# kopacja/rho2sdf.jl

Measured on NVIDIA B200. Metric: sdf_voxels_per_sec, higher is better.
Workload: dtype f64

## Files before the change

### include/r2s.h

```cpp
#ifndef R2S_H
#define R2S_H
#include <stddef.h>
#include <stdint.h>
#ifdef __cplusplus
extern "C" {
#endif

typedef struct r2s_ctx r2s_ctx;

typedef struct r2s_params {
  double rho_t;
  double delta_factor;
  int32_t remove_artifacts;
  double artifact_threshold;
  double artifact_min_ratio;
  int32_t rbf_interp;
  int32_t smooth;
  double rbf_cut;
  double target_volume;
  int32_t final_volume;
} r2s_params;

typedef struct r2s_report {
  int64_t n_solid, n_crossing, n_active, n_pairs, n_not_converged, n_newton_iters;
  int64_t n_flipped;
  int32_t cg_iters, bisections;
  float th, volume;
  float ms_bin, ms_project, ms_assemble, ms_sign, ms_cc, ms_rbf_prep, ms_cg, ms_lsf, ms_threshold, ms_fine, ms_volume, ms_total;
  int64_t launches;
  int64_t collectives;
  float cg_probe[4];
  int64_t n_pairs_pruned;
  float ms_solve, ms_scan;
} r2s_report;

int r2s_create(r2s_ctx **ctx, int device, void *stream);
void r2s_destroy(r2s_ctx *ctx);
const char *r2s_last_error(r2s_ctx *ctx);
void r2s_default_params(r2s_params *p);
int r2s_last_report(r2s_ctx *ctx, r2s_report *rep);

int r2s_set_mesh(r2s_ctx *ctx, int nen, int64_t nnp, const double *X, int64_t nel, const int64_t *IEN);
int r2s_set_grid(r2s_ctx *ctx, const double amin[3], const double amax[3], const int64_t N[3], double cell_size);

int r2s_mesh_volume(r2s_ctx *ctx, const double *rho_e, double *V_domain, double *V_frac);
int r2s_nodal_densities(r2s_ctx *ctx, const double *rho_e, double *rho_n);
int r2s_isocontour_volume(r2s_ctx *ctx, const double *rho_n, double threshold, double *volume);
int r2s_find_threshold(r2s_ctx *ctx, const double *rho_n, double target_volume, double rtol, int maxit, double *rho_t);

int r2s_eval_distances(r2s_ctx *ctx, const double *rho_n, double rho_t, double delta_factor, double *dist, double *xp);
int r2s_sign_detection(r2s_ctx *ctx, const double *rho_n, double rho_t, double *signs);
int r2s_remove_artifacts(r2s_ctx *ctx, double *sdf, double threshold, double min_component_ratio, int64_t *flipped);
int r2s_rbf_smoothing(r2s_ctx *ctx, const double *sdf, int is_interp, int smooth, double rbf_cut, double target_volume,
                      float *fine_sdf, float *th, float *volume);
int r2s_volume_from_sdf(r2s_ctx *ctx, const float *sdf, int64_t nx, int64_t ny, int64_t nz, float edge, float iso, int quad_order, double *volume);

int r2s_pipeline(r2s_ctx *ctx, const r2s_params *p, const double *rho_n, double *sdf_dists, float *fine_sdf, r2s_report *rep);
int r2s_upload_nodal_densities(r2s_ctx *ctx, const double *rho_n);
int r2s_pipeline_resident(r2s_ctx *ctx, const r2s_params *p, r2s_report *rep);
int r2s_download_sdf(r2s_ctx *ctx, double *sdf_dists);
int r2s_download_fine_sdf(r2s_ctx *ctx, float *fine_sdf);
int r2s_result_ptrs_dev(r2s_ctx *ctx, void **sdf_dev, void **fine_sdf_dev);

// ... 41 lines not shown
```

### rho2sdf.jl_b200/__init__.py

```python
import ctypes as C
import math
import os

import numpy as np

__all__ = ["HEX8", "TET4", "Rho2sdfOptions", "Mesh", "Grid", "getMesh_AABB", "generateGridPoints", "noninteractive_sdf_grid_setup",
           "DenseInNodes", "find_threshold_for_volume", "calculate_isocontour_volume", "evalDistances", "Sign_Detection",
           "remove_sdf_artifacts", "RBFs_smoothing", "calculate_volume_from_sdf", "rho2sdf", "rho2sdf_hex8", "rho2sdf_tet4",
           "exportSdfToVTI", "export_device_result_to_vti", "read_vti", "read_pvti", "MultiContext", "FineGrid", "R2SError", "slab_partition", "init_slab_comm", "broadcast_unique_id", "load_library", "library_path", "Params", "Report", "Context"]

_HERE = os.path.dirname(os.path.abspath(__file__))
_LIB = None


class R2SError(RuntimeError):
    pass


class HEX8:
    nen = 8


class TET4:
    nen = 4


class Params(C.Structure):
    _fields_ = [("rho_t", C.c_double), ("delta_factor", C.c_double), ("remove_artifacts", C.c_int32), ("artifact_threshold", C.c_double),
                ("artifact_min_ratio", C.c_double), ("rbf_interp", C.c_int32), ("smooth", C.c_int32), ("rbf_cut", C.c_double),
# ... 70 lines not shown
    L.r2s_multi_context.restype = vp
    L.r2s_multi_set_mesh.argtypes = [vp, C.c_int, C.c_int64, vp, C.c_int64, vp]
    L.r2s_multi_set_grid.argtypes = [vp, vp, vp, vp, C.c_double]
    L.r2s_multi_slab_planes.argtypes = [vp, vp]
    L.r2s_multi_set_rebalance.argtypes = [vp, C.c_int]
    L.r2s_multi_pipeline.argtypes = [vp, C.POINTER(Params), vp, vp, vp, C.POINTER(Report)]
    L.r2s_multi_export_vti.argtypes = [vp, C.c_char_p, C.c_char_p, C.c_int]
    L.r2s_pin_host.argtypes = [vp, C.c_size_t]
    L.r2s_unpin_host.argtypes = [vp]
    L.r2s_write_vti_host.argtypes = [C.c_char_p, C.c_char_p, vp, C.c_int, C.c_int64, C.c_int64, C.c_int64, vp, vp]
    L.r2s_measure_fma_peak.argtypes = [vp, C.c_int, dp]
    _LIB = L
    return L


def _f64(a):
    return np.ascontiguousarray(a, dtype=np.float64)


def _ptr(a):
    return a.ctypes.data_as(C.c_void_p)


class _BorrowedContext:

    def __init__(self, lib, h):
        self.lib, self.h = lib, C.c_void_p(h)

    def check(self, rc):
        if rc != 0:
            raise R2SError(self.lib.r2s_last_error(self.h).decode())

    def close(self):
        pass

    def report(self):
        r = Report()
        self.lib.r2s_last_report(self.h, C.byref(r))
        return r


class MultiContext:

    def __init__(self, devices):
        self.lib = load_library()
        self.h = C.c_void_p()
        ids = (C.c_int * len(devices))(*[int(d) for d in devices])
        rc = self.lib.r2s_multi_create(C.byref(self.h), ids, len(devices))
        if rc != 0 or not self.h:
            raise R2SError("r2s_multi_create failed (rc=%d): no usable CUDA device / no peer access -- this library has no CPU fallback" % rc)
        self.n = len(devices)

    def check(self, rc):
        if rc != 0:
            raise R2SError(self.lib.r2s_multi_last_error(self.h).decode())

    def slab(self, r=0):
        return _BorrowedContext(self.lib, self.lib.r2s_multi_context(self.h, int(r)))

    def slab_planes(self):
        cuts = np.zeros(self.n + 1, dtype=np.int64)
        self.check(self.lib.r2s_multi_slab_planes(self.h, _ptr(cuts)))
# ... 20 lines not shown
        if rc != 0 or not self.h:
            raise R2SError("r2s_create failed (rc=%d): no usable CUDA device -- this library has no CPU fallback" % rc)
        self._keep = []

    def check(self, rc):
        if rc != 0:
            raise R2SError(self.lib.r2s_last_error(self.h).decode())

    def close(self):
        if self.h:
            self.lib.r2s_destroy(self.h)
            self.h = C.c_void_p()

    def __del__(self):
        try:
            self.close()
        except Exception:
            pass

    def report(self):
        r = Report()
        self.lib.r2s_last_report(self.h, C.byref(r))
        return r


def slab_partition(nz_points, world, plane_cost=None, min_planes=3):
    nz_points, world = int(nz_points), int(world)
    if world < 1 or nz_points < world * (min_planes if world > 1 else 1):
        raise R2SError("cannot cut %d planes into %d slabs" % (nz_points, world))
    if plane_cost is None:
        base, rem = divmod(nz_points, world)
        out, k = [], 0
        for r in range(world):
            n = base + (1 if r < rem else 0)
            out.append((k, k + n))
            k += n
        return out
    c = np.maximum(np.asarray(plane_cost, dtype=np.float64), 1e-12)
    if c.shape != (nz_points,):
        raise R2SError("plane_cost must have one entry per plane")
    cum = np.concatenate([[0.0], np.cumsum(c)])
    cuts = [0]
    for r in range(1, world):
        k = int(np.searchsorted(cum, cum[-1] * r / world))
        k = max(k, cuts[-1] + min_planes)
        k = min(k, nz_points - (world - r) * min_planes)
# ... 380 lines not shown
```

### rho2sdf.jl_b200/csrc/r2s_api.cu

```cuda
#include <math.h>
#include <stdlib.h>
#include <string.h>
#include <new>
#include "r2s_common.cuh"


extern "C" {

int r2s_create(r2s_ctx **out, int device, void *stream) {
  if (!out) return 1;
  *out = nullptr;
  int ndev = 0;
  if (cudaGetDeviceCount(&ndev) != cudaSuccess || ndev == 0 || device < 0 || device >= ndev) return 2;
  r2s_ctx *ctx = new (std::nothrow) r2s_ctx();
  if (!ctx) return 3;
  ctx->device = device;
  memset(&ctx->rep, 0, sizeof(ctx->rep));
  if (cudaSetDevice(device) != cudaSuccess) { delete ctx; return 4; }
  if (stream) { ctx->stream = (cudaStream_t)stream; ctx->own_stream = false; }
  else { if (cudaStreamCreateWithFlags(&ctx->stream, cudaStreamNonBlocking) != cudaSuccess) { delete ctx; return 5; } ctx->own_stream = true; }
  for (int i = 0; i < 16; i++) cudaEventCreate(&ctx->ev[i]);
  for (int i = 0; i < 5; i++) { cudaEventCreate(&ctx->ev_probe[i]); cudaEventCreate(&ctx->ev_k[i]); }
  cudaStreamCreateWithFlags(&ctx->copy_stream, cudaStreamNonBlocking);
  for (int i = 0; i < 64; i++) cudaEventCreateWithFlags(&ctx->ev_copy[i], cudaEventDisableTiming);
// ... 12 lines not shown
  r2s_comm_destroy(ctx);
  DevBuf *all[] = {&ctx->X, &ctx->IEN32, &ctx->ine_ptr, &ctx->ine_el, &ctx->fbnd, &ctx->ezr, &ctx->ebox, &ctx->rho_e, &ctx->rho_n, &ctx->gtab_d, &ctx->gtab_i, &ctx->cls, &ctx->act_flag,
                   &ctx->act_idx, &ctx->act_rec, &ctx->cnt_a, &ctx->cnt_b, &ctx->keys, &ctx->keys_alt, &ctx->tile_ptr, &ctx->tile_faces, &ctx->face_tiles, &ctx->fc_list, &ctx->tri_cnt, &ctx->tri_rec, &ctx->pairbuf, &ctx->pairxp, &ctx->cubtmp,
                   &ctx->counters, &ctx->box_rec, &ctx->plist, &ctx->dist, &ctx->xp, &ctx->sdf, &ctx->signs, &ctx->s_rng, &ctx->s_el, &ctx->s_cnt, &ctx->s_keys, &ctx->s_keys_alt, &ctx->s_tile_ptr,
                   &ctx->cc_label, &ctx->cc_size, &ctx->cc_scal, &ctx->cc_bits, &ctx->cc_bits_all, &ctx->cc_gsz, &ctx->cc_seen, &ctx->f_s, &ctx->f_w, &ctx->f_r, &ctx->f_u, &ctx->f_c, &ctx->f_lsf, &ctx->f_fine, &ctx->f_part,
                   &ctx->f_scal, &ctx->cutlist, &ctx->slablist, &ctx->v_part, &ctx->vlist[0], &ctx->vlist[1], &ctx->vent[0], &ctx->vent[1], &ctx->vrec, &ctx->bis_state, &ctx->lat_xs, &ctx->lat_cell, &ctx->lat_map, &ctx->lat_info, &ctx->lat_pt};
  for (DevBuf *b : all) b->release();
  for (int i = 0; i < 16; i++) cudaEventDestroy(ctx->ev[i]);
  for (int i = 0; i < 5; i++) { cudaEventDestroy(ctx->ev_probe[i]); cudaEventDestroy(ctx->ev_k[i]); }
  for (int i = 0; i < 64; i++) cudaEventDestroy(ctx->ev_copy[i]);
  for (int i = 0; i < 2; i++) cudaEventDestroy(ctx->ev_done[i]);
  if (ctx->copy_stream) cudaStreamDestroy(ctx->copy_stream);
  if (ctx->rb_host) cudaFreeHost(ctx->rb_host);
  if (ctx->own_stream) cudaStreamDestroy(ctx->stream);
  delete ctx;
}
const char *r2s_last_error(r2s_ctx *ctx) { return ctx ? ctx->err.c_str() : "r2s: no context (no CUDA device?)"; }

void r2s_default_params(r2s_params *p) {
  p->rho_t = 0.5; p->delta_factor = 1.1; p->remove_artifacts = 1; p->artifact_threshold = 0.0; p->artifact_min_ratio = 0.01;
  p->rbf_interp = 1; p->smooth = 1; p->rbf_cut = 1e-3; p->target_volume = 0.0; p->final_volume = 1;
}
int r2s_last_report(r2s_ctx *ctx, r2s_report *rep) { if (!ctx || !rep) return 1; *rep = ctx->rep; return 0; }

int r2s_set_mesh(r2s_ctx *ctx, int nen, int64_t nnp, const double *X, int64_t nel, const int64_t *IEN) {
  if (!ctx) return 1;
  if (nen != 8 && nen != 4) FAIL("r2s_set_mesh: nen must be 8 (HEX8) or 4 (TET4)");
  if (nnp <= 0 || nel <= 0 || !X || !IEN) FAIL("r2s_set_mesh: empty mesh");
  if (nel * nen >= (1ll << 31) || nnp >= (1ll << 31)) FAIL("r2s_set_mesh: mesh too large for 32-bit connectivity");
  CK(cudaSetDevice(ctx->device));
  for (i64 t = 0; t < nel * nen; t++) if (IEN[t] < 1 || IEN[t] > nnp) FAIL("r2s_set_mesh: IEN entry out of range (expected 1-based node ids)");
  ctx->have_sdf = ctx->have_fine = false;
  ctx->nen = nen; ctx->nes = nen == 8 ? 6 : 4; ctx->nsn = nen == 8 ? 4 : 3; ctx->nnp = nnp; ctx->nel = nel;
  CK(ctx->X.reserve(sizeof(double) * 3 * (size_t)nnp));
  CK(ctx->IEN32.reserve(sizeof(int) * (size_t)(nel * nen)));
  CK(cudaMemcpyAsync(ctx->X.p, X, sizeof(double) * 3 * (size_t)nnp, cudaMemcpyHostToDevice, ctx->stream));
  if (r2s_mesh_upload_ien(ctx, IEN)) return 1;
  CK(ctx->rho_e.reserve(sizeof(double) * (size_t)nel));
  CK(ctx->rho_n.reserve(sizeof(double) * (size_t)nnp));
  if (r2s_mesh_build_tables(ctx)) return 1;
  return r2s_mesh_build_lattice(ctx);
}

int r2s_set_grid(r2s_ctx *ctx, const double amin[3], const double amax[3], const int64_t N[3], double cell) {
  if (!ctx) return 1;
  CK(cudaSetDevice(ctx->device));
// ... 300 lines not shown
```

### rho2sdf.jl_b200/csrc/r2s_common.cuh

```cuda
#pragma once
#include <cuda_runtime.h>
#include <stdint.h>
#include <stdio.h>
#include <string>
#include <vector>
#include "../../include/r2s.h"

typedef long long i64;
typedef unsigned long long u64;

#define R2S_BIG 1.0e10

#define TILE_X 8
#define TILE_Y 8
#define TILE_Z 4
#define TILE_VOX (TILE_X * TILE_Y * TILE_Z)

struct DevBuf {
  void *p = nullptr;
  size_t cap = 0;
  cudaError_t reserve(size_t bytes) {
    if (bytes <= cap) return cudaSuccess;
    if (p) cudaFree(p);
    p = nullptr; cap = 0;
// ... 58 lines not shown
  i64 nnp = 0, nel = 0;
  DevBuf X, IEN32, ine_ptr, ine_el, fbnd, ezr;
  DevBuf ebox; i64 n_box = 0;
  bool lattice = false; int lat_nd[3] = {0, 0, 0}, lat_off[3] = {0, 0, 0}; i64 lat_ncell = 0;
  DevBuf lat_xs, lat_cell, lat_map, lat_info, lat_pt;
  DevBuf rho_e, rho_n;

  bool has_grid = false;
  GridDev g;
  i64 k0 = 0, k1 = 0;
  const float *skip_flag = nullptr;
  LocalGroup *lg = nullptr;
  void *comm = nullptr; int rank = 0, nranks = 1; i64 collectives = 0; std::vector<int> slab_k0;
  bool p2p = false; void *p2p_box = nullptr; void *p2p_peer_box[64]; void **p2p_peer_box_dev = nullptr; unsigned p2p_seq = 0;
  void *p2p_c_local = nullptr; void *p2p_c_peer[2] = {nullptr, nullptr}; unsigned p2p_halo_seq = 0; i64 p2p_ops = 0;
  DevBuf gtab_d, gtab_i;
  std::vector<double> h_pc[3];

  DevBuf cls, act_flag, act_idx, act_rec, cnt_a, cnt_b, keys, keys_alt, tile_ptr, tile_faces, face_tiles, fc_list, tri_cnt, tri_rec, pairbuf, pairxp, cubtmp, counters, box_rec, plist;
  DevBuf dist, xp, sdf, signs;
  DevBuf s_rng, s_el, s_cnt, s_keys, s_keys_alt, s_tile_ptr;
  DevBuf cc_label, cc_size, cc_scal, cc_bits, cc_bits_all, cc_gsz, cc_seen;
  DevBuf f_s, f_w, f_r, f_u, f_c, f_lsf, f_fine, f_part, f_scal, cutlist, slablist, vlist[2], vent[2], vrec, bis_state;
  int smooth_last = 1;
  bool have_sdf = false, have_fine = false;

  DevBuf v_part;
};

#define CK(call)                                                                                   \
  do {                                                                                             \
    cudaError_t _e = (call);                                                                       \
    if (_e != cudaSuccess) {                                                                       \
      char _b[512];                                                                                \
      snprintf(_b, sizeof(_b), "%s:%d: %s -> %s", __FILE__, __LINE__, #call, cudaGetErrorString(_e)); \
      ctx->err = _b;                                                                               \
      return 1;                                                                                    \
    }                                                                                              \
  } while (0)

#define FAIL(msg)           \
  do {                      \
    ctx->err = (msg);       \
    return 1;               \
  } while (0)

// ... 70 lines not shown
```

### rho2sdf.jl_b200/csrc/r2s_rbf.cu

```cuda
#include <float.h>
#include <stdlib.h>
#include <algorithm>
#include <cuda.h>
#include "r2s_common.cuh"
#include "r2s_tables.cuh"
#include "r2s_p2p.cuh"
#include "r2s_volq.cuh"

__global__ void __launch_bounds__(256) k_to_f32(i64 n, i64 v0, int nx, int px, const double *__restrict__ sdf, float *__restrict__ s, unsigned *__restrict__ maxbits) {
  __shared__ float red[8];
  float a = -1.0f;
  const i64 row0 = v0 / nx;
  for (i64 v = blockIdx.x * (i64)blockDim.x + threadIdx.x; v < n; v += (i64)gridDim.x * blockDim.x) {
    const i64 row = v / nx; const int i = (int)(v - row * nx);
    float f = (float)sdf[v0 + v]; s[(row0 + row) * px + i] = f; float af = fabsf(f); if (af < 1.0e9f) a = fmaxf(a, af);
  }
  for (int o = 16; o > 0; o >>= 1) a = fmaxf(a, __shfl_down_sync(0xffffffffu, a, o));
  if ((threadIdx.x & 31) == 0) red[threadIdx.x >> 5] = a;
  __syncthreads();
  if (threadIdx.x == 0) {
    for (int i = 1; i < 8; i++) a = fmaxf(a, red[i]);
    if (a >= 0.0f) atomicMax(maxbits, __float_as_uint(a) + 1u);
  }
}
// ... 279 lines not shown
  for (i64 v = blockIdx.x * (i64)blockDim.x + threadIdx.x; v < n; v += (i64)gridDim.x * blockDim.x) s += (double)a[v] * (double)a[v];
  for (int o = 16; o > 0; o >>= 1) s += __shfl_down_sync(0xffffffffu, s, o);
  if ((threadIdx.x & 31) == 0) red[threadIdx.x >> 5] = s;
  __syncthreads();
  if (threadIdx.x == 0) { double t = 0; for (int i = 0; i < (int)(blockDim.x >> 5); i++) t += red[i]; partial[blockIdx.x] = t; }
}

__global__ void __launch_bounds__(256) k_minmax(i64 n, int nx, int px, const float *__restrict__ a, unsigned *__restrict__ mm) {
  __shared__ float rlo[8], rhi[8];
  float lo = INFINITY, hi = -INFINITY;
  for (i64 v = blockIdx.x * (i64)blockDim.x + threadIdx.x; v < n; v += (i64)gridDim.x * blockDim.x) { if ((int)(v % px) < nx) { float x = a[v]; lo = fminf(lo, x); hi = fmaxf(hi, x); } }
  for (int o = 16; o > 0; o >>= 1) { lo = fminf(lo, __shfl_down_sync(0xffffffffu, lo, o)); hi = fmaxf(hi, __shfl_down_sync(0xffffffffu, hi, o)); }
  if ((threadIdx.x & 31) == 0) { rlo[threadIdx.x >> 5] = lo; rhi[threadIdx.x >> 5] = hi; }
  __syncthreads();
  if (threadIdx.x == 0) {
    for (int i = 1; i < 8; i++) { lo = fminf(lo, rlo[i]); hi = fmaxf(hi, rhi[i]); }
    unsigned bl = __float_as_uint(lo), bh = __float_as_uint(hi);
    bl = (bl & 0x80000000u) ? ~bl : (bl | 0x80000000u); bh = (bh & 0x80000000u) ? ~bh : (bh | 0x80000000u);
    atomicMin(&mm[0], bl); atomicMax(&mm[1], bh);
  }
}
static inline float ordered_to_float(unsigned b) { b = (b & 0x80000000u) ? (b & 0x7fffffffu) : ~b; float f; memcpy(&f, &b, 4); return f; }

__device__ __forceinline__ void vol_sum_flush(u64 local, u64 *__restrict__ acc) {
  __shared__ u64 s_w[2][8];
  u64 s[2] = {local & 0xffffffffull, local >> 32};
  for (int o = 16; o > 0; o >>= 1) { s[0] += __shfl_down_sync(0xffffffffu, s[0], o); s[1] += __shfl_down_sync(0xffffffffu, s[1], o); }
  if ((threadIdx.x & 31) == 0) { s_w[0][threadIdx.x >> 5] = s[0]; s_w[1][threadIdx.x >> 5] = s[1]; }
  __syncthreads();
  if (threadIdx.x == 0) {
    u64 a = 0, b = 0;
    for (int w = 0; w < (int)(blockDim.x >> 5); w++) { a += s_w[0][w]; b += s_w[1][w]; }
    if (a) atomicAdd(&acc[2], a);
    if (b) atomicAdd(&acc[7], b);
  }
}
__global__ void __launch_bounds__(128) k_vol_cut(int nx, int ny, int px, const float *__restrict__ sdf, float th, float iso, const int *__restrict__ cutlist, int cutcap,
                                                 GaussF G, u64 *__restrict__ acc) {
  const int ncut = (int)min((u64)cutcap, acc[1]);
  const int nthr = gridDim.x * blockDim.x;
  const i64 sxy = (i64)px * ny;
  u64 local = 0;
  for (int base = blockIdx.x * blockDim.x; base < ncut; base += nthr) {
    const int idx = base + threadIdx.x;
    if (idx < ncut) {
      const i64 c = cutlist[idx];
// ... 139 lines not shown
    int cutcap = (int)(ctx->cutlist.cap / sizeof(int));
    CK(cudaMemsetAsync(acc, 0, sizeof(u64) * 8, st));
    vol_march<false>(st, nx, ny, px, 0, nz - 1, sdf, iso, iso, iso, nullptr, nullptr, 0, acc, ctx->cutlist.as<int>(), cutcap); LAUNCH_CHECK();
    if (order == 9) k_vol_cut<<<148 * 16, 128, 0, st>>>(nx, ny, px, sdf, 0.0f, iso, ctx->cutlist.as<int>(), cutcap, G9, acc);
    else {
      GaussTab t = gauss_legendre_host(order); GaussNF G; G.n = order;
      for (int q = 0; q < 32; q++) { G.x[q] = q < order ? (float)t.x[q] : 0.0f; G.w[q] = q < order ? (float)t.w[q] : 0.0f; }
      k_vol_cut_n<<<148 * 16, 128, 0, st>>>(nx, ny, px, sdf, 0.0f, iso, ctx->cutlist.as<int>(), cutcap, G, acc);
    }
    LAUNCH_CHECK();
    u64 h[8];
    if (r2s_readback(ctx, h, acc, sizeof(h))) return 1;
    if ((i64)h[1] > cutcap) {
      CK(ctx->cutlist.reserve(sizeof(int) * (size_t)(h[1] + h[1] / 2 + 1024)));
      continue;
    }
    float ev = edge * edge * edge, jac = ev / 8.0f;
    *vol = (double)h[0] * (double)ev + vol_fixed_value(h[2], h[7]) * (double)jac;
    return 0;
  }
  FAIL("calculate_volume_from_sdf: cut-cell list overflow");
}
struct VRec { float c[8]; };
struct VCache { float part, th_e, margin; int pad; };
struct BisState {
  float lo, hi, th, th_prev; int nb, have_prev, done, skip; float skipf; int cur; double v, eps, target; float ev, jac; unsigned long long n_eval;
};
__device__ __forceinline__ void bis_begin(BisState *S, u64 *acc) {
  if (S->done) { S->skip = 1; S->skipf = 1.0f; return; }
  const float th = (S->lo + S->hi) / 2;
  S->th = th;
  const int skip = (S->have_prev && th == S->th_prev) ? 1 : 0;
  S->skip = skip; S->skipf = skip ? 1.0f : 0.0f;
  if (!skip) { acc[0] = 0; acc[1] = 0; acc[2] = 0; acc[7] = 0; acc[4 + (1 - S->cur)] = 0; }
}
__device__ __forceinline__ void bis_end(BisState *S, const u64 *acc, const u64 *red) {
  if (S->done) return;
  if (!S->skip) {
    S->v = fma((double)red[0], (double)S->ev, __dmul_rn(vol_fixed_value(red[2], red[3]), (double)S->jac));
    S->cur = 1 - S->cur; S->n_eval += acc[1];
  }
  const float cur = (float)S->v;
  S->eps = fabs(S->target - (double)cur);
  if ((double)cur > S->target) S->lo = S->th; else S->hi = S->th;
  S->nb++; S->have_prev = 1; S->th_prev = S->th;
  if (!(S->nb < 40 && S->eps > 1.0e-4)) S->done = 1;
}
#define VL_U 4
__global__ void __launch_bounds__(256) k_vl_step(const BisState *__restrict__ S, VAct *l0, VAct *l1, i64 out_cap, int use_cache, u64 *__restrict__ acc, const VCache *__restrict__ cache,
                                                 int2 *__restrict__ evlist, i64 ev_cap) {
  if (S->skip) return;
  const int icur = S->cur;
  const VAct *__restrict__ in = icur ? l1 : l0; VAct *__restrict__ out = icur ? l0 : l1;
  const u64 *n_in_ptr = acc + 4 + icur; u64 *n_out_ptr = acc + 4 + (1 - icur);
  const float lo = S->lo, hi = S->hi, th = S->th;
  __shared__ VAct s_keep[8][WS_CAP];
  __shared__ int2 s_ev[8][WS_CAP];
  const i64 n_in = (i64)*n_in_ptr;
  const int lane = threadIdx.x & 31, warp = threadIdx.x >> 5;
  int nfull = 0, nperm = 0, nkq = 0, neq = 0; u64 local = 0;
  for (i64 t0 = ((i64)blockIdx.x * blockDim.x + (threadIdx.x & ~31)) * VL_U; t0 < n_in; t0 += (i64)gridDim.x * blockDim.x * VL_U) {
    VAct e[VL_U];
#pragma unroll
    for (int u = 0; u < VL_U; u++) {
      const i64 t = t0 + u * 32 + lane;
      if (t < n_in) { const int4 q = __ldcs(reinterpret_cast<const int4 *>(in) + t); e[u].id = q.x; e[u].mn = __int_as_float(q.y); e[u].mx = __int_as_float(q.z); e[u].rec = q.w; }
      else { e[u].id = 0; e[u].mn = INFINITY; e[u].mx = INFINITY; e[u].rec = -1; }
    }
    float4 r[VL_U];
#pragma unroll
    for (int u = 0; u < VL_U; u++) {
      r[u] = make_float4(0.f, 0.f, 0.f, 0.f);
      const bool cached = use_cache && e[u].rec >= 0 && !(e[u].mn >= hi) && !(e[u].mx < lo) && !(e[u].mx < th) && !(e[u].mn >= th);
      if (cached) r[u] = __ldg(reinterpret_cast<const float4 *>(cache) + e[u].rec);
    }
#pragma unroll
    for (int u = 0; u < VL_U; u++) {
      const bool valid = t0 + u * 32 + lane < n_in;
      bool keep = false, miss = false, fresh = false;
      if (valid) {
        if (e[u].mn >= hi) nperm++;
        else if (e[u].mx < lo) {}
        else {
          keep = true;
          if (!(e[u].mx < th)) {
            if (e[u].mn >= th) nfull++;
            else if (e[u].rec < 0) { miss = true; fresh = true; }
            else if (use_cache && fabsf(th - r[u].y) * 1.00001f < r[u].z) vol_cell_add(local, r[u].x);
            else miss = true;
          }
        }
      }
      const unsigned mf = __ballot_sync(0xffffffffu, fresh);
      if (mf) {
        int base = 0;
        if (lane == 0) base = (int)atomicAdd(&acc[6], (u64)__popc(mf));
        base = __shfl_sync(0xffffffffu, base, 0);
        if (fresh) e[u].rec = base + __popc(mf & ((1u << lane) - 1));
      }
      ws_push<VAct>(s_keep[warp], nkq, keep, e[u], out, n_out_ptr, out_cap, lane);
      ws_push<int2>(s_ev[warp], neq, miss, make_int2(e[u].rec | (fresh ? (int)0x80000000 : 0), e[u].id), evlist, &acc[1], ev_cap, lane);
    }
  }
  ws_flush<VAct>(s_keep[warp], nkq, out, n_out_ptr, out_cap, lane);
  ws_flush<int2>(s_ev[warp], neq, evlist, &acc[1], ev_cap, lane);
  for (int o = 16; o > 0; o >>= 1) { nfull += __shfl_down_sync(0xffffffffu, nfull, o); nperm += __shfl_down_sync(0xffffffffu, nperm, o); }
  if (lane == 0) { if (nfull) atomicAdd(&acc[0], (u64)nfull); if (nperm) atomicAdd(&acc[3], (u64)nperm); }
  vol_sum_flush(local, acc);
}
__global__ void __launch_bounds__(128) k_vl_eval(const BisState *__restrict__ S, VRec *__restrict__ recs, VCache *__restrict__ cache, const int2 *__restrict__ evlist, int nx, int ny,
                                                 int px, const float *__restrict__ sdf, GaussF G, u64 *__restrict__ acc) {
  if (S->skip) return;
  const float th = S->th;
  const int nev = (int)acc[1];
  const int nthr = gridDim.x * blockDim.x;
  u64 local = 0;
  for (int base = blockIdx.x * blockDim.x; base < nev; base += nthr) {
    const int idx = base + threadIdx.x;
    if (idx < nev) {
      const int2 q = evlist[idx];
      VRec &e = recs[q.x & 0x7fffffff];
      float c[8];
      if (q.x < 0) {
        const i64 cpl = (i64)(nx - 1) * (ny - 1), sxy = (i64)px * ny;
        const int i = q.y % (nx - 1), j = (q.y / (nx - 1)) % (ny - 1), k = (int)(q.y / cpl);
        const i64 b = ((i64)k * ny + j) * px + i;
        c[0] = sdf[b]; c[1] = sdf[b + 1]; c[2] = sdf[b + px]; c[3] = sdf[b + px + 1];
        c[4] = sdf[b + sxy]; c[5] = sdf[b + sxy + 1]; c[6] = sdf[b + sxy + px]; c[7] = sdf[b + sxy + px + 1];
        float4 *d = reinterpret_cast<float4 *>(e.c);
        d[0] = make_float4(c[0], c[1], c[2], c[3]); d[1] = make_float4(c[4], c[5], c[6], c[7]);
      } else {
        const float4 *d = reinterpret_cast<const float4 *>(e.c), a = d[0], b = d[1];
        c[0] = a.x; c[1] = a.y; c[2] = a.z; c[3] = a.w; c[4] = b.x; c[5] = b.y; c[6] = b.z; c[7] = b.w;
      }
#pragma unroll
      for (int a = 0; a < 8; a++) c[a] = c[a] - th;
      const float amax = fmaxf(fmaxf(fmaxf(fabsf(c[0]), fabsf(c[1])), fmaxf(fabsf(c[2]), fabsf(c[3]))), fmaxf(fmaxf(fabsf(c[4]), fabsf(c[5])), fmaxf(fabsf(c[6]), fabsf(c[7]))));
      float m;
      const float part = cut_cell_quad9<true>(c, G, 0.0f, &m);
      VCache w; w.part = part; w.th_e = th; w.margin = m - 1.0e-5f * amax; w.pad = 0;
      cache[q.x & 0x7fffffff] = w;
      vol_cell_add(local, part);
    }
  }
  vol_sum_flush(local, acc);
}
__device__ __forceinline__ void vol_pack(const u64 *__restrict__ acc, int cutcap, u64 *__restrict__ red, const BisState *S) {
  if (S && S->skip) return;
  red[0] = acc[0] + acc[3]; red[1] = acc[1] > (u64)cutcap ? 1 : 0; red[2] = acc[2]; red[3] = acc[7];
}
__global__ void k_vol_pack(const u64 *__restrict__ acc, int cutcap, u64 *__restrict__ red, const BisState *S) { vol_pack(acc, cutcap, red, S); }
__global__ void k_bis_turn(BisState *S, u64 *acc, u64 *red, int what) {
  if (what & 4) vol_pack(acc, 0x7fffffff, red, S);
  if (what & 2) bis_end(S, acc, red);
  if (what & 1) bis_begin(S, acc);
}
struct VolBisect {
  const float *sdf; int nx, ny, px, kc0, kc1; float edge; int step, cur; i64 n_cur, n_eval; u64 *acc;
};
static int vol_bisect_begin(r2s_ctx *ctx, VolBisect &vb, const float *sdf, int nx, int ny, int nz, int px, int kc0, int kc1, float edge) {
  i64 ncell = (i64)(nx - 1) * (ny - 1) * (nz - 1);
  if (ncell >= (1ll << 31)) FAIL("LS_Threshold: grid too large for 32-bit cell ids");
  CK(ctx->f_scal.reserve(512));
  vb.sdf = sdf; vb.nx = nx; vb.ny = ny; vb.px = px; vb.kc0 = kc0; vb.kc1 = kc1; vb.edge = edge; vb.step = 0; vb.cur = 0; vb.n_eval = 0;
  vb.n_cur = (i64)(nx - 1) * (ny - 1) * (i64)(kc1 - kc0);
  vb.acc = (u64 *)((char *)ctx->f_scal.p + 128);
  CK(cudaMemsetAsync(vb.acc, 0, sizeof(u64) * 12, ctx->stream));
  return 0;
}
static int vol_bisect_step(r2s_ctx *ctx, VolBisect &vb, float lo, float hi, float th, double *vol) {
  cudaStream_t st = ctx->stream;
  static const GaussF G9 = gauss9f();
  const i64 n_all = (i64)(vb.nx - 1) * (vb.ny - 1) * (i64)(vb.kc1 - vb.kc0);
  vb.step++;
  const bool emit = vb.step == 3;
  if (emit) CK(ctx->vent[0].reserve(sizeof(VAct) * (size_t)(n_all + 1)));
  u64 h[6];
  for (int attempt = 0; attempt < 2; attempt++) {
    int cutcap = (int)(ctx->cutlist.cap / sizeof(int));
    CK(cudaMemsetAsync(vb.acc, 0, sizeof(u64) * 8, st));
    u64 *nout = vb.acc + 4;
    if (!emit) vol_march<false>(st, vb.nx, vb.ny, vb.px, vb.kc0, vb.kc1, vb.sdf, lo, hi, th, nullptr, nullptr, 0, vb.acc, ctx->cutlist.as<int>(), cutcap);
    else vol_march<true>(st, vb.nx, vb.ny, vb.px, vb.kc0, vb.kc1, vb.sdf, lo, hi, th, ctx->vent[0].as<VAct>(), nout, n_all + 1, vb.acc, ctx->cutlist.as<int>(), cutcap);
    LAUNCH_CHECK();
    k_vol_cut<<<148 * 16, 128, 0, st>>>(vb.nx, vb.ny, vb.px, vb.sdf, th, 0.0f, ctx->cutlist.as<int>(), cutcap, G9, vb.acc); LAUNCH_CHECK();
    u64 *red = vb.acc + 8, hr[4];
    k_vol_pack<<<1, 1, 0, st>>>(vb.acc, cutcap, red, nullptr); LAUNCH_CHECK();
    if (r2s_allreduce(ctx, red, 4, 1)) return 1;
    {
      u64 hall[12];
      if (r2s_readback(ctx, hall, vb.acc, sizeof(hall))) return 1;
      for (int q = 0; q < 6; q++) h[q] = hall[q];
      for (int q = 0; q < 4; q++) hr[q] = hall[8 + q];
    }
    if (hr[1] != 0) {
      if ((i64)h[1] > cutcap) CK(ctx->cutlist.reserve(sizeof(int) * (size_t)(h[1] + h[1] / 2 + 1024)));
      continue;
    }
    if (emit) {
      vb.cur = 0; vb.n_cur = (i64)h[4];
      CK(ctx->vrec.reserve((sizeof(VRec) + sizeof(VCache)) * (size_t)(vb.n_cur + 1)));
    }
    vb.n_eval += (i64)h[1];
    float ev = vb.edge * vb.edge * vb.edge, jac = ev / 8.0f;
    *vol = (double)hr[0] * (double)ev + vol_fixed_value(hr[2], hr[3]) * (double)jac;
    return 0;
  }
  FAIL("LS_Threshold: cut-cell list overflow");
}
static int vol_bisect_finish(r2s_ctx *ctx, VolBisect &vb, float &lo, float &hi, float &th, double &v, double &eps, int &nb, float th_prev, double target) {
  cudaStream_t st = ctx->stream;
  static const GaussF G9 = gauss9f();
  CK(ctx->vent[1].reserve(sizeof(VAct) * (size_t)(vb.n_cur + 1)));
  CK(ctx->vlist[1].reserve(sizeof(int2) * (size_t)(vb.n_cur + 1)));
  CK(ctx->bis_state.reserve(256));
  BisState h; memset(&h, 0, sizeof(h));
  h.lo = lo; h.hi = hi; h.th = th; h.th_prev = th_prev; h.nb = nb; h.have_prev = 1; h.done = 0; h.cur = 0; h.v = v; h.eps = eps; h.target = target;
  h.ev = vb.edge * vb.edge * vb.edge; h.jac = h.ev / 8.0f;
  BisState *S = ctx->bis_state.as<BisState>();
  CK(cudaMemcpyAsync(S, &h, sizeof(h), cudaMemcpyHostToDevice, st));
  const int grid = (int)std::min<i64>(std::max<i64>(cdiv(vb.n_cur, 256 * VL_U), 1), 148 * 8);
  VRec *recs = ctx->vrec.as<VRec>(); VCache *cache = reinterpret_cast<VCache *>(recs + (vb.n_cur + 1));
  u64 *red = vb.acc + 8;
  ctx->skip_flag = &S->skipf;
  const bool single = ctx->nranks == 1;
  k_bis_turn<<<1, 1, 0, st>>>(S, vb.acc, red, 1); LAUNCH_CHECK();
  for (int step = nb; step < 40; step++) {
    const int next = step + 1 < 40 ? 1 : 0;
    k_vl_step<<<grid, 256, 0, st>>>(S, ctx->vent[0].as<VAct>(), ctx->vent[1].as<VAct>(), vb.n_cur + 1, ctx->knobs.vol_cache, vb.acc, cache, ctx->vlist[1].as<int2>(), vb.n_cur + 1); LAUNCH_CHECK();
    k_vl_eval<<<148 * 16, 128, 0, st>>>(S, recs, cache, ctx->vlist[1].as<int2>(), vb.nx, vb.ny, vb.px, vb.sdf, G9, vb.acc); LAUNCH_CHECK();
    if (single) { k_bis_turn<<<1, 1, 0, st>>>(S, vb.acc, red, 4 | 2 | next); LAUNCH_CHECK(); }
    else {
      k_bis_turn<<<1, 1, 0, st>>>(S, vb.acc, red, 4); LAUNCH_CHECK();
      if (r2s_allreduce(ctx, red, 4, 1)) { ctx->skip_flag = nullptr; return 1; }
      k_bis_turn<<<1, 1, 0, st>>>(S, vb.acc, red, 2 | next); LAUNCH_CHECK();
    }
  }
  ctx->skip_flag = nullptr;
  if (r2s_readback(ctx, &h, S, sizeof(h))) return 1;
  lo = h.lo; hi = h.hi; th = h.th; v = h.v; eps = h.eps; nb = h.nb; vb.n_eval += (i64)h.n_eval;
  return 0;
}
int r2s_dev_volume_from_sdf(r2s_ctx *ctx, const float *sdf_dev, i64 nx, i64 ny, i64 nz, float edge, float iso, int order, double *vol) {
  if (order < 1 || order > 32) FAIL("calculate_volume_from_sdf: detailed_quad_order must be between 1 and 32");
  CK(ctx->cutlist.reserve(sizeof(int) * 1024));
  return volume_dev(ctx, sdf_dev, (int)nx, (int)ny, (int)nz, (int)nx, edge, iso, order, vol);
}

struct TapTable { int n[8]; int off[8][96]; };
__constant__ float c_tapw[8][96];
__constant__ TapTable c_taps;
#define FN_X 32
#define FN_Y 4
#define FN_Z 4
template <int SM>
__global__ void __launch_bounds__(FN_X *FN_Y *FN_Z) k_fine_eval(int nx, int ny, int nz, int px, int fx, int fy, int fz, int kf0, const float *__restrict__ w, float th, float *__restrict__ out) {
  constexpr int CX = FN_X / SM + 6, CY = FN_Y / SM + 6 + 1, CZ = FN_Z / SM + 6 + 1;
  __shared__ float sm[CZ][CY][CX + 1];
  const int fbx = blockIdx.x * FN_X, fby = blockIdx.y * FN_Y, fbz = kf0 + blockIdx.z * FN_Z;
  const int cbx = fbx / SM - 3, cby = fby / SM - 3, cbz = fbz / SM - 3;
  for (int t = threadIdx.x; t < CX * CY * CZ; t += blockDim.x) {
    int lx = t % CX, ly = (t / CX) % CY, lz = t / (CX * CY);
    int gx = cbx + lx, gy = cby + ly, gz = cbz + lz;
// ... 248 lines not shown
  }
  LAUNCH_CHECK();
  if (r2s_halo_exchange_f32(ctx, lsf, pl, k0, k1, nz, 0, 1)) return 1;
  unsigned init_mm[2] = {0xffffffffu, 0u};
  CK(cudaMemcpyAsync(ubits + 2, init_mm, sizeof(init_mm), cudaMemcpyHostToDevice, st));
  k_minmax<<<(int)std::min<i64>(cdiv(nown, 256), CG_BLOCKS), 256, 0, st>>>(nown, nx, px, lsf + o_lo, ubits + 2); LAUNCH_CHECK();
  if (r2s_group_start(ctx)) return 1;
  if (r2s_allreduce(ctx, ubits + 2, 1, 3)) return 1;
  if (r2s_allreduce(ctx, ubits + 3, 1, 2)) return 1;
  if (r2s_group_end(ctx)) return 1;
  unsigned hmm[2];
  if (r2s_readback(ctx, hmm, ubits + 2, sizeof(hmm))) return 1;
  CK(cudaEventRecord(ctx->ev[7], st));
  float lo = ordered_to_float(hmm[0]), hi = ordered_to_float(hmm[1]);
  float edge;
  {
    float a = (float)g.amin[0], b = (float)g.amax[0];
    float x0 = a, x1 = (nx > 1) ? (float)((double)a + 1.0 * (((double)b - (double)a) / (double)(nx - 1))) : a;
    if (nx == 2) x1 = b;
    float ex = x1 - x0; edge = sqrtf(ex * ex);
  }
  double eps = 1.0; int nb = 0; float th = 0.0f; double v = 0.0; bool have_prev = false; float th_prev = 0.0f;
  VolBisect vb;
  if (vol_bisect_begin(ctx, vb, lsf, nx, ny, nz, px, k0, std::min(k1, nz - 1), edge)) return 1;
  while (nb < 40 && eps > 1.0e-4) {
    th = (lo + hi) / 2;
    if (!(have_prev && th == th_prev)) { if (vol_bisect_step(ctx, vb, lo, hi, th, &v)) return 1; }
    have_prev = true; th_prev = th;
    float cur = (float)v;
    eps = fabs(target - (double)cur);
    if ((double)cur > target) lo = th; else hi = th;
    nb++;
    if (vb.step == 3 && nb < 40 && eps > 1.0e-4) { if (vol_bisect_finish(ctx, vb, lo, hi, th, v, eps, nb, th_prev, target)) return 1; break; }
  }
  ctx->rep.bisections = nb;
  float tho = -th;
  CK(cudaEventRecord(ctx->ev[13], st));
  if (upload_taps(ctx, smooth, rbf_cut, g.cell)) return 1;
  {
    const int chunk = ctx->async_fine_host ? 32 : (k1 - k0);
    for (int c0 = k0; c0 < k1; c0 += chunk) {
      const int c1 = std::min(c0 + chunk, k1);
      const int f0 = smooth * c0, f1 = (c1 < nz) ? smooth * c1 : fz;
      if (smooth == 1) {
        dim3 fgrid(cdiv(fx, FN_X), cdiv(fy, FN_Y), cdiv(f1 - f0, FN_Z));
        k_fine_eval<1><<<fgrid, FN_X * FN_Y * FN_Z, 0, st>>>(nx, ny, nz, px, fx, fy, f1, f0, wgt, tho, ctx->f_fine.as<float>());
// ... 38 lines not shown
```

### rho2sdf.jl_b200/csrc/r2s_volq.cuh

```cuda
#pragma once
#include <math.h>

#if defined(__CUDACC__)
#define R2S_HD __host__ __device__ __forceinline__
#else
#define R2S_HD inline
#endif

struct GaussF { float x[9]; float w[9]; };
struct F2 { float x, y; };

R2S_HD float q_mul(float a, float b) {
#if defined(__CUDA_ARCH__)
  return __fmul_rn(a, b);
#else
  return a * b;
#endif
}
R2S_HD float q_sub(float a, float b) {
#if defined(__CUDA_ARCH__)
  return __fsub_rn(a, b);
#else
  return a - b;
#endif
}
R2S_HD F2 q_mul2(F2 a, F2 b) {
#if defined(__CUDA_ARCH__)
  unsigned long long xa = *reinterpret_cast<unsigned long long *>(&a), xb = *reinterpret_cast<unsigned long long *>(&b), r;
  asm("mul.rn.f32x2 %0, %1, %2;" : "=l"(r) : "l"(xa), "l"(xb));
  return *reinterpret_cast<F2 *>(&r);
#else
  return F2{a.x * b.x, a.y * b.y};
#endif
}
R2S_HD F2 q_fma2(F2 a, F2 b, F2 c) {
#if defined(__CUDA_ARCH__)
  unsigned long long xa = *reinterpret_cast<unsigned long long *>(&a), xb = *reinterpret_cast<unsigned long long *>(&b), xc = *reinterpret_cast<unsigned long long *>(&c), r;
  asm("fma.rn.f32x2 %0, %1, %2, %3;" : "=l"(r) : "l"(xa), "l"(xb), "l"(xc));
  return *reinterpret_cast<F2 *>(&r);
#else
  return F2{fmaf(a.x, b.x, c.x), fmaf(a.y, b.y, c.y)};
#endif
}
R2S_HD float q_unit(float x) { return q_mul(x + 1.0f, 0.5f); }

template <bool MARGIN>
R2S_HD float cut_cell_quad9(const float c[8], const GaussF &G, float iso, float *mabs) {
  const F2 f00 = {c[0], c[4]}, f10 = {c[1], c[5]}, f01 = {c[2], c[6]}, f11 = {c[3], c[7]};
  float part = 0.0f, m = INFINITY;
#if defined(__CUDA_ARCH__)
#pragma unroll 1
#endif
  for (int iq = 0; iq < 9; iq++) {
    const float xi = q_unit(G.x[iq]), xm = 1.0f - xi;
    const F2 vxi = {xi, xi}, vxm = {xm, xm};
    const F2 a = q_fma2(f10, vxi, q_mul2(f00, vxm));
    const F2 b = q_fma2(f11, vxi, q_mul2(f01, vxm));
#if defined(__CUDA_ARCH__)
#pragma unroll
#endif
    for (int jq = 0; jq < 9; jq++) {
      const float eta = q_unit(G.x[jq]), em = 1.0f - eta;
      const F2 cc = q_fma2(b, F2{eta, eta}, q_mul2(a, F2{em, em}));
      const float c0 = cc.x, dc = q_sub(cc.y, cc.x), wij = q_mul(G.w[iq], G.w[jq]);
#if defined(__CUDA_ARCH__)
#pragma unroll
#endif
      for (int kq = 0; kq < 9; kq += 2) {
        float ps[2];
        if (kq + 1 < 9) {
          const F2 p = q_fma2(F2{dc, dc}, F2{q_unit(G.x[kq]), q_unit(G.x[kq + 1])}, F2{c0, c0});
          ps[0] = p.x; ps[1] = p.y;
        } else {
          ps[0] = fmaf(dc, q_unit(G.x[kq]), c0); ps[1] = 0.0f;
        }
#if defined(__CUDA_ARCH__)
#pragma unroll
#endif
        for (int h = 0; h < 2; h++) {
          if (kq + h >= 9) break;
          if (ps[h] >= iso) part = fmaf(wij, G.w[kq + h], part);
          if (MARGIN) m = fminf(m, fabsf(ps[h]));
        }
      }
    }
  }
  if (MARGIN) *mabs = m;
  return part;
}

R2S_HD void vol_cell_add(unsigned long long &local, float part) {
  local += (unsigned long long)llrint((double)part * 137438953472.0 );
}
R2S_HD double vol_fixed_value(unsigned long long s0w, unsigned long long s1w) {
  const unsigned long long lo = s0w + (s1w << 32), hi = (s1w >> 32) + (lo < s0w ? 1ull : 0ull);
  if (hi == 0) return (double)lo / 137438953472.0;
  int sh = 0;
  while (sh < 64 && (hi >> sh) != 0) sh++;
  const unsigned long long t = (lo >> sh) | (hi << (64 - sh)) | ((lo & ((1ull << sh) - 1)) != 0 ? 1ull : 0ull);
  return ldexp((double)t, sh - 37);
}
```

Before: 10.82 billion.

## Freeze bracket-stable cut cells and use directional cache margins in volume bisection

The volume-threshold bisection cache now stores separate upward and downward margins, so a cached quadrature result is reused whenever the threshold shift stays inside the margin on its side. Cells whose cached value holds at both bracket ends are frozen. They leave the active list and their volume goes into a separate accumulator, which shrinks the list and the re-evaluation work in later steps. The step and eval kernels also exit early when their input count is zero. The change adds per-iteration diagnostic counters exposed through a new API, and reductions now go through a generic CTA add covering five values, which costs a little extra atomic and shared-memory work.

```diff
diff --git a/include/r2s.h b/include/r2s.h
--- a/include/r2s.h
+++ b/include/r2s.h
@@ -39,6 +39,7 @@
 const char *r2s_last_error(r2s_ctx *ctx);
 void r2s_default_params(r2s_params *p);
 int r2s_last_report(r2s_ctx *ctx, r2s_report *rep);
+int r2s_threshold_counts(r2s_ctx *ctx, int64_t *counts);
 
 int r2s_set_mesh(r2s_ctx *ctx, int nen, int64_t nnp, const double *X, int64_t nel, const int64_t *IEN);
 int r2s_set_grid(r2s_ctx *ctx, const double amin[3], const double amax[3], const int64_t N[3], double cell_size);
diff --git a/rho2sdf.jl_b200/__init__.py b/rho2sdf.jl_b200/__init__.py
--- a/rho2sdf.jl_b200/__init__.py
+++ b/rho2sdf.jl_b200/__init__.py
@@ -4,7 +4,7 @@
 
 import numpy as np
 
-__all__ = ["HEX8", "TET4", "Rho2sdfOptions", "Mesh", "Grid", "getMesh_AABB", "generateGridPoints", "noninteractive_sdf_grid_setup",
+__all__ = ["HEX8", "TET4", "THRESHOLD_COUNT_COLUMNS", "Rho2sdfOptions", "Mesh", "Grid", "getMesh_AABB", "generateGridPoints", "noninteractive_sdf_grid_setup",
            "DenseInNodes", "find_threshold_for_volume", "calculate_isocontour_volume", "evalDistances", "Sign_Detection",
            "remove_sdf_artifacts", "RBFs_smoothing", "calculate_volume_from_sdf", "rho2sdf", "rho2sdf_hex8", "rho2sdf_tet4",
            "exportSdfToVTI", "export_device_result_to_vti", "read_vti", "read_pvti", "MultiContext", "FineGrid", "R2SError", "slab_partition", "init_slab_comm", "broadcast_unique_id", "load_library", "library_path", "Params", "Report", "Context"]
@@ -121,6 +121,9 @@
     return a.ctypes.data_as(C.c_void_p)
 
 
+THRESHOLD_COUNT_COLUMNS = ("list", "queued", "fresh", "full", "empty", "frozen")
+
+
 class _BorrowedContext:
 
     def __init__(self, lib, h):
@@ -137,6 +140,11 @@
         r = Report()
         self.lib.r2s_last_report(self.h, C.byref(r))
         return r
+
+    def threshold_counts(self):
+        c = np.zeros((40, 6), dtype=np.int64)
+        self.check(self.lib.r2s_threshold_counts(self.h, _ptr(c)))
+        return c
 
 
 class MultiContext:
@@ -203,6 +211,11 @@
         r = Report()
         self.lib.r2s_last_report(self.h, C.byref(r))
         return r
+
+    def threshold_counts(self):
+        c = np.zeros((40, 6), dtype=np.int64)
+        self.check(self.lib.r2s_threshold_counts(self.h, _ptr(c)))
+        return c
 
 
 def slab_partition(nz_points, world, plane_cost=None, min_planes=3):
diff --git a/rho2sdf.jl_b200/csrc/r2s_api.cu b/rho2sdf.jl_b200/csrc/r2s_api.cu
--- a/rho2sdf.jl_b200/csrc/r2s_api.cu
+++ b/rho2sdf.jl_b200/csrc/r2s_api.cu
@@ -58,6 +58,11 @@
   p->rbf_interp = 1; p->smooth = 1; p->rbf_cut = 1e-3; p->target_volume = 0.0; p->final_volume = 1;
 }
 int r2s_last_report(r2s_ctx *ctx, r2s_report *rep) { if (!ctx || !rep) return 1; *rep = ctx->rep; return 0; }
+int r2s_threshold_counts(r2s_ctx *ctx, int64_t *counts) {
+  if (!ctx || !counts) return 1;
+  memcpy(counts, ctx->bis_cnt, sizeof(ctx->bis_cnt));
+  return 0;
+}
 
 int r2s_set_mesh(r2s_ctx *ctx, int nen, int64_t nnp, const double *X, int64_t nel, const int64_t *IEN) {
   if (!ctx) return 1;
diff --git a/rho2sdf.jl_b200/csrc/r2s_common.cuh b/rho2sdf.jl_b200/csrc/r2s_common.cuh
--- a/rho2sdf.jl_b200/csrc/r2s_common.cuh
+++ b/rho2sdf.jl_b200/csrc/r2s_common.cuh
@@ -104,6 +104,7 @@
   DevBuf s_rng, s_el, s_cnt, s_keys, s_keys_alt, s_tile_ptr;
   DevBuf cc_label, cc_size, cc_scal, cc_bits, cc_bits_all, cc_gsz, cc_seen;
   DevBuf f_s, f_w, f_r, f_u, f_c, f_lsf, f_fine, f_part, f_scal, cutlist, slablist, vlist[2], vent[2], vrec, bis_state;
+  unsigned long long bis_cnt[40][6] = {};
   int smooth_last = 1;
   bool have_sdf = false, have_fine = false;
 
diff --git a/rho2sdf.jl_b200/csrc/r2s_rbf.cu b/rho2sdf.jl_b200/csrc/r2s_rbf.cu
--- a/rho2sdf.jl_b200/csrc/r2s_rbf.cu
+++ b/rho2sdf.jl_b200/csrc/r2s_rbf.cu
@@ -325,6 +325,24 @@
 }
 static inline float ordered_to_float(unsigned b) { b = (b & 0x80000000u) ? (b & 0x7fffffffu) : ~b; float f; memcpy(&f, &b, 4); return f; }
 
+template <int N>
+__device__ __forceinline__ void cta_add(u64 (&v)[N], u64 *const (&dst)[N]) {
+  __shared__ u64 s_w[N][8];
+#pragma unroll
+  for (int q = 0; q < N; q++)
+    for (int o = 16; o > 0; o >>= 1) v[q] += __shfl_down_sync(0xffffffffu, v[q], o);
+  if ((threadIdx.x & 31) == 0)
+#pragma unroll
+    for (int q = 0; q < N; q++) s_w[q][threadIdx.x >> 5] = v[q];
+  __syncthreads();
+  if (threadIdx.x == 0)
+#pragma unroll
+    for (int q = 0; q < N; q++) {
+      u64 a = 0;
+      for (int w = 0; w < (int)(blockDim.x >> 5); w++) a += s_w[q][w];
+      if (a) atomicAdd(dst[q], a);
+    }
+}
 __device__ __forceinline__ void vol_sum_flush(u64 local, u64 *__restrict__ acc) {
   __shared__ u64 s_w[2][8];
   u64 s[2] = {local & 0xffffffffull, local >> 32};
@@ -510,9 +528,12 @@
   FAIL("calculate_volume_from_sdf: cut-cell list overflow");
 }
 struct VRec { float c[8]; };
-struct VCache { float part, th_e, margin; int pad; };
+struct VCache { float part, th_e, m_up, m_dn; };
+enum { BC_LIST, BC_QUEUED, BC_FRESH, BC_FULL, BC_EMPTY, BC_FROZEN, BC_N };
 struct BisState {
   float lo, hi, th, th_prev; int nb, have_prev, done, skip; float skipf; int cur; double v, eps, target; float ev, jac; unsigned long long n_eval;
+  unsigned long long seen_full, seen_rec;
+  unsigned long long cnt[40][BC_N];
 };
 __device__ __forceinline__ void bis_begin(BisState *S, u64 *acc) {
   if (S->done) { S->skip = 1; S->skipf = 1.0f; return; }
@@ -520,12 +541,16 @@
   S->th = th;
   const int skip = (S->have_prev && th == S->th_prev) ? 1 : 0;
   S->skip = skip; S->skipf = skip ? 1.0f : 0.0f;
-  if (!skip) { acc[0] = 0; acc[1] = 0; acc[2] = 0; acc[7] = 0; acc[4 + (1 - S->cur)] = 0; }
+  if (!skip) { acc[0] = 0; acc[1] = 0; acc[2] = 0; acc[7] = 0; acc[14] = 0; acc[4 + (1 - S->cur)] = 0; }
 }
 __device__ __forceinline__ void bis_end(BisState *S, const u64 *acc, const u64 *red) {
   if (S->done) return;
   if (!S->skip) {
     S->v = fma((double)red[0], (double)S->ev, __dmul_rn(vol_fixed_value(red[2], red[3]), (double)S->jac));
+    unsigned long long *c = S->cnt[S->nb];
+    c[BC_LIST] = acc[4 + S->cur]; c[BC_QUEUED] = acc[1]; c[BC_FRESH] = acc[6] - S->seen_rec; c[BC_FULL] = acc[3] - S->seen_full; c[BC_FROZEN] = acc[14];
+    c[BC_EMPTY] = c[BC_LIST] - acc[4 + (1 - S->cur)] - c[BC_FULL] - c[BC_FROZEN];
+    S->seen_rec = acc[6]; S->seen_full = acc[3];
     S->cur = 1 - S->cur; S->n_eval += acc[1];
   }
   const float cur = (float)S->v;
@@ -537,16 +562,16 @@
 #define VL_U 4
 __global__ void __launch_bounds__(256) k_vl_step(const BisState *__restrict__ S, VAct *l0, VAct *l1, i64 out_cap, int use_cache, u64 *__restrict__ acc, const VCache *__restrict__ cache,
                                                  int2 *__restrict__ evlist, i64 ev_cap) {
-  if (S->skip) return;
   const int icur = S->cur;
+  const u64 *n_in_ptr = acc + 4 + icur; u64 *n_out_ptr = acc + 4 + (1 - icur);
+  const i64 n_in = (i64)*n_in_ptr;
+  if (S->skip || n_in == 0) return;
   const VAct *__restrict__ in = icur ? l1 : l0; VAct *__restrict__ out = icur ? l0 : l1;
-  const u64 *n_in_ptr = acc + 4 + icur; u64 *n_out_ptr = acc + 4 + (1 - icur);
   const float lo = S->lo, hi = S->hi, th = S->th;
   __shared__ VAct s_keep[8][WS_CAP];
   __shared__ int2 s_ev[8][WS_CAP];
-  const i64 n_in = (i64)*n_in_ptr;
   const int lane = threadIdx.x & 31, warp = threadIdx.x >> 5;
-  int nfull = 0, nperm = 0, nkq = 0, neq = 0; u64 local = 0;
+  int nfull = 0, nperm = 0, nkq = 0, neq = 0; u64 local = 0, frozen = 0, nfrozen = 0;
   for (i64 t0 = ((i64)blockIdx.x * blockDim.x + (threadIdx.x & ~31)) * VL_U; t0 < n_in; t0 += (i64)gridDim.x * blockDim.x * VL_U) {
     VAct e[VL_U];
 #pragma unroll
@@ -571,10 +596,12 @@
         else if (e[u].mx < lo) {}
         else {
           keep = true;
-          if (!(e[u].mx < th)) {
+          if (use_cache && e[u].rec >= 0 && e[u].mn < lo && e[u].mx >= hi && vol_cache_holds(lo, r[u].y, r[u].z, r[u].w) && vol_cache_holds(hi, r[u].y, r[u].z, r[u].w)) {
+            keep = false; nfrozen++; vol_cell_add(frozen, r[u].x);
+          } else if (!(e[u].mx < th)) {
             if (e[u].mn >= th) nfull++;
             else if (e[u].rec < 0) { miss = true; fresh = true; }
-            else if (use_cache && fabsf(th - r[u].y) * 1.00001f < r[u].z) vol_cell_add(local, r[u].x);
+            else if (use_cache && vol_cache_holds(th, r[u].y, r[u].z, r[u].w)) vol_cell_add(local, r[u].x);
             else miss = true;
           }
         }
@@ -594,13 +621,15 @@
   ws_flush<int2>(s_ev[warp], neq, evlist, &acc[1], ev_cap, lane);
   for (int o = 16; o > 0; o >>= 1) { nfull += __shfl_down_sync(0xffffffffu, nfull, o); nperm += __shfl_down_sync(0xffffffffu, nperm, o); }
   if (lane == 0) { if (nfull) atomicAdd(&acc[0], (u64)nfull); if (nperm) atomicAdd(&acc[3], (u64)nperm); }
-  vol_sum_flush(local, acc);
+  u64 v[5] = {local & 0xffffffffull, local >> 32, frozen & 0xffffffffull, frozen >> 32, nfrozen};
+  u64 *const dst[5] = {&acc[2], &acc[7], &acc[12], &acc[13], &acc[14]};
+  cta_add(v, dst);
 }
 __global__ void __launch_bounds__(128) k_vl_eval(const BisState *__restrict__ S, VRec *__restrict__ recs, VCache *__restrict__ cache, const int2 *__restrict__ evlist, int nx, int ny,
                                                  int px, const float *__restrict__ sdf, GaussF G, u64 *__restrict__ acc) {
-  if (S->skip) return;
+  const int nev = (int)acc[1];
+  if (S->skip || nev == 0) return;
   const float th = S->th;
-  const int nev = (int)acc[1];
   const int nthr = gridDim.x * blockDim.x;
   u64 local = 0;
   for (int base = blockIdx.x * blockDim.x; base < nev; base += nthr) {
@@ -623,10 +652,10 @@
       }
 #pragma unroll
       for (int a = 0; a < 8; a++) c[a] = c[a] - th;
-      const float amax = fmaxf(fmaxf(fmaxf(fabsf(c[0]), fabsf(c[1])), fmaxf(fabsf(c[2]), fabsf(c[3]))), fmaxf(fmaxf(fabsf(c[4]), fabsf(c[5])), fmaxf(fabsf(c[6]), fabsf(c[7]))));
-      float m;
-      const float part = cut_cell_quad9<true>(c, G, 0.0f, &m);
-      VCache w; w.part = part; w.th_e = th; w.margin = m - 1.0e-5f * amax; w.pad = 0;
+      float m_in, m_out;
+      VCache w; w.part = cut_cell_quad9<true>(c, G, 0.0f, &m_in, &m_out); w.th_e = th;
+      vol_cache_margins(c, m_in, m_out, &w.m_up, &w.m_dn);
+      const float part = w.part;
       cache[q.x & 0x7fffffff] = w;
       vol_cell_add(local, part);
     }
@@ -635,7 +664,7 @@
 }
 __device__ __forceinline__ void vol_pack(const u64 *__restrict__ acc, int cutcap, u64 *__restrict__ red, const BisState *S) {
   if (S && S->skip) return;
-  red[0] = acc[0] + acc[3]; red[1] = acc[1] > (u64)cutcap ? 1 : 0; red[2] = acc[2]; red[3] = acc[7];
+  red[0] = acc[0] + acc[3]; red[1] = acc[1] > (u64)cutcap ? 1 : 0; red[2] = acc[2] + acc[12]; red[3] = acc[7] + acc[13];
 }
 __global__ void k_vol_pack(const u64 *__restrict__ acc, int cutcap, u64 *__restrict__ red, const BisState *S) { vol_pack(acc, cutcap, red, S); }
 __global__ void k_bis_turn(BisState *S, u64 *acc, u64 *red, int what) {
@@ -644,7 +673,7 @@
   if (what & 1) bis_begin(S, acc);
 }
 struct VolBisect {
-  const float *sdf; int nx, ny, px, kc0, kc1; float edge; int step, cur; i64 n_cur, n_eval; u64 *acc;
+  const float *sdf; int nx, ny, px, kc0, kc1; float edge; int step, cur; i64 n_cur, n_eval; u64 *acc; u64 n_perm;
 };
 static int vol_bisect_begin(r2s_ctx *ctx, VolBisect &vb, const float *sdf, int nx, int ny, int nz, int px, int kc0, int kc1, float edge) {
   i64 ncell = (i64)(nx - 1) * (ny - 1) * (nz - 1);
@@ -653,7 +682,7 @@
   vb.sdf = sdf; vb.nx = nx; vb.ny = ny; vb.px = px; vb.kc0 = kc0; vb.kc1 = kc1; vb.edge = edge; vb.step = 0; vb.cur = 0; vb.n_eval = 0;
   vb.n_cur = (i64)(nx - 1) * (ny - 1) * (i64)(kc1 - kc0);
   vb.acc = (u64 *)((char *)ctx->f_scal.p + 128);
-  CK(cudaMemsetAsync(vb.acc, 0, sizeof(u64) * 12, ctx->stream));
+  CK(cudaMemsetAsync(vb.acc, 0, sizeof(u64) * 15, ctx->stream));
   return 0;
 }
 static int vol_bisect_step(r2s_ctx *ctx, VolBisect &vb, float lo, float hi, float th, double *vol) {
@@ -686,7 +715,7 @@
       continue;
     }
     if (emit) {
-      vb.cur = 0; vb.n_cur = (i64)h[4];
+      vb.cur = 0; vb.n_cur = (i64)h[4]; vb.n_perm = h[3];
       CK(ctx->vrec.reserve((sizeof(VRec) + sizeof(VCache)) * (size_t)(vb.n_cur + 1)));
     }
     vb.n_eval += (i64)h[1];
@@ -701,8 +730,9 @@
   static const GaussF G9 = gauss9f();
   CK(ctx->vent[1].reserve(sizeof(VAct) * (size_t)(vb.n_cur + 1)));
   CK(ctx->vlist[1].reserve(sizeof(int2) * (size_t)(vb.n_cur + 1)));
-  CK(ctx->bis_state.reserve(256));
+  CK(ctx->bis_state.reserve(sizeof(BisState)));
   BisState h; memset(&h, 0, sizeof(h));
+  h.seen_full = vb.n_perm;
   h.lo = lo; h.hi = hi; h.th = th; h.th_prev = th_prev; h.nb = nb; h.have_prev = 1; h.done = 0; h.cur = 0; h.v = v; h.eps = eps; h.target = target;
   h.ev = vb.edge * vb.edge * vb.edge; h.jac = h.ev / 8.0f;
   BisState *S = ctx->bis_state.as<BisState>();
@@ -727,6 +757,8 @@
   ctx->skip_flag = nullptr;
   if (r2s_readback(ctx, &h, S, sizeof(h))) return 1;
   lo = h.lo; hi = h.hi; th = h.th; v = h.v; eps = h.eps; nb = h.nb; vb.n_eval += (i64)h.n_eval;
+  static_assert(sizeof(h.cnt) == sizeof(ctx->bis_cnt), "r2s_ctx::bis_cnt mirrors BisState::cnt");
+  memcpy(ctx->bis_cnt, h.cnt, sizeof(h.cnt));
   return 0;
 }
 int r2s_dev_volume_from_sdf(r2s_ctx *ctx, const float *sdf_dev, i64 nx, i64 ny, i64 nz, float edge, float iso, int order, double *vol) {
@@ -1021,6 +1053,7 @@
   }
   double eps = 1.0; int nb = 0; float th = 0.0f; double v = 0.0; bool have_prev = false; float th_prev = 0.0f;
   VolBisect vb;
+  memset(ctx->bis_cnt, 0, sizeof(ctx->bis_cnt));
   if (vol_bisect_begin(ctx, vb, lsf, nx, ny, nz, px, k0, std::min(k1, nz - 1), edge)) return 1;
   while (nb < 40 && eps > 1.0e-4) {
     th = (lo + hi) / 2;
diff --git a/rho2sdf.jl_b200/csrc/r2s_volq.cuh b/rho2sdf.jl_b200/csrc/r2s_volq.cuh
--- a/rho2sdf.jl_b200/csrc/r2s_volq.cuh
+++ b/rho2sdf.jl_b200/csrc/r2s_volq.cuh
@@ -1,5 +1,6 @@
 #pragma once
 #include <math.h>
+#include <string.h>
 
 #if defined(__CUDACC__)
 #define R2S_HD __host__ __device__ __forceinline__
@@ -42,12 +43,28 @@
   return F2{fmaf(a.x, b.x, c.x), fmaf(a.y, b.y, c.y)};
 #endif
 }
+R2S_HD unsigned q_bits(float a) {
+#if defined(__CUDA_ARCH__)
+  return __float_as_uint(a);
+#else
+  unsigned u; memcpy(&u, &a, 4); return u;
+#endif
+}
+R2S_HD float q_float(unsigned u) {
+#if defined(__CUDA_ARCH__)
+  return __uint_as_float(u);
+#else
+  float a; memcpy(&a, &u, 4); return a;
+#endif
+}
 R2S_HD float q_unit(float x) { return q_mul(x + 1.0f, 0.5f); }
 
 template <bool MARGIN>
-R2S_HD float cut_cell_quad9(const float c[8], const GaussF &G, float iso, float *mabs) {
+R2S_HD float cut_cell_quad9(const float c[8], const GaussF &G, float iso, float *m_in, float *m_out) {
   const F2 f00 = {c[0], c[4]}, f10 = {c[1], c[5]}, f01 = {c[2], c[6]}, f11 = {c[3], c[7]};
-  float part = 0.0f, m = INFINITY;
+  float part = 0.0f;
+  unsigned mi = 0x7f800000u;
+  int mo = 0x7f800000;
 #if defined(__CUDA_ARCH__)
 #pragma unroll 1
 #endif
@@ -80,13 +97,32 @@
         for (int h = 0; h < 2; h++) {
           if (kq + h >= 9) break;
           if (ps[h] >= iso) part = fmaf(wij, G.w[kq + h], part);
-          if (MARGIN) m = fminf(m, fabsf(ps[h]));
+          if (MARGIN) { const unsigned b = q_bits(ps[h]); mi = mi < b ? mi : b; mo = mo < (int)b ? mo : (int)b; }
         }
       }
     }
   }
-  if (MARGIN) *mabs = m;
+  if (MARGIN) { *m_in = q_float(mi); *m_out = mo < 0 ? fabsf(q_float((unsigned)mo)) : INFINITY; }
   return part;
+}
+template <bool MARGIN>
+R2S_HD float cut_cell_quad9(const float c[8], const GaussF &G, float iso, float *mabs) {
+  float m_in, m_out;
+  const float part = cut_cell_quad9<MARGIN>(c, G, iso, &m_in, &m_out);
+  if (MARGIN) *mabs = fminf(m_in, m_out);
+  return part;
+}
+
+R2S_HD void vol_cache_margins(const float c[8], float m_in, float m_out, float *m_up, float *m_dn) {
+  float amax = 0.0f;
+  for (int a = 0; a < 8; a++) amax = fmaxf(amax, fabsf(c[a]));
+  const float tol = q_mul(1.0e-5f, amax);
+  *m_up = q_sub(m_out > tol ? m_in : 0.0f, tol);
+  *m_dn = q_sub(m_in > tol ? m_out : 0.0f, tol);
+}
+R2S_HD bool vol_cache_holds(float th, float th_e, float m_up, float m_dn) {
+  const float d = q_sub(th, th_e);
+  return q_mul(fabsf(d), 1.00001f) < (d > 0.0f ? m_up : m_dn);
 }
 
 R2S_HD void vol_cell_add(unsigned long long &local, float part) {
```

Result: faster. 10.97 billion, median of 6 (+1.4%).
